# alan-turing-institute/rPSMF

Measured on AMD Instinct MI355X. Metric: PSMF filter timesteps/sec at d=100k r=32, higher is better.
Workload: dtype f64; 1 GPU; PSMF full filter, random-walk dynamics, d=100000 r=32 T=10000 synthetic Gaussian series, rows sharded over 1 GPU(s); d=100000, d_per_gpu=100000, r=32, T=10000, store_y_pred=True, engine=block

## Files before the change

rpsmf_amd/csrc/psmf_blk3.hip:

```cpp
#pragma once
#include "psmf_block.h"
#include "psmf_sweep.h"
#include "psmf_ns.hip"
#include "psmf_dyn.hip"
#include "psmf_wave.h"

namespace psmf {

constexpr int F3_NT = 512;
constexpr int F3_S = 34;
constexpr int F3_MAXIT = 12;

template <int MODE>
struct F3Mask {
  static constexpr bool full = MODE == 0;
  static constexpr bool small = MODE == 2;
  bool c1, r1[4], dg[4];
};
#define F3_VALID(mk, ti, tj, q) ((mk).full || ((mk).small ? ((ti) == 0 && (tj) == 0 && (mk).r1[q] && (mk).c1) \
                                                          : (((ti) == 0 || (mk).r1[q]) && ((tj) == 0 || (mk).c1))))
#define F3_DIAG(mk, ti, tj, q) (((ti) == (tj)) && (mk).dg[q])

enum { F3_KAPPA = 0, F3_N, F3_INVN, F3_EE, F3_IOM, F3_Q, F3_IQ, F3_PSCALE, F3_NSC = 16 };

// ... 12 lines not shown
  double* sc;
  double* nrm;
  double* hv;
  double* gp;
  double* tr;
  double* sab;
  double* sal;
  double* sbe;
  float* s32;
  double* rowbufX;
  double* rowbufY;
  int* errflag;
  long long* tick;
  long long* acc;
  long long* hand;
};

constexpr int F3_AS = 48;

inline size_t blk_filter3_lds_bytes() {
  const size_t doubles = (size_t)RB * RB + 2 * (size_t)RB * F3_AS + 2 * 32 * F3_S + 8 * RM + 2;
  return (doubles * 8 + 15) & ~(size_t)15;
}

struct F3Blk {
  long long k0;
  int nb, last;
  double* Acoef;
  double* Bcoef;
  const double* XG;
  const double* Aprev;
  int from_lds, to_lds;
};

enum { F3C_IQW = 0, F3C_IOM, F3C_PSCALE, F3C_Q, F3C_RHO, F3C_LAM, F3C_PHI, F3C_OMEGA, F3C_EE, F3C_S, F3C_ETA, F3C_N };
struct F3Carry {
  double* Xc;
  float* Xa;
  double* G;
  double* W;
  double* V;
  double* sc;
};
__device__ __forceinline__ F3Carry f3_carry(const F3Lds& L) {
  F3Carry c;
  c.Xc = L.dump;
  c.Xa = L.dumpP;
  c.G = L.dump + 4 * 8 * 64;
  c.W = L.dump + 6 * 8 * 64;
  c.V = L.img;
  c.sc = L.img + 16 * 64;
  return c;
}
__device__ __forceinline__ int f3_carry_xa(const int role, const int e, const int lane) { return (((e >> 3) * 4 + role) * 8 + (e & 7)) * 64 + lane; }

__device__ __forceinline__ void f3_ns_dump(DevState* st, const int role, const int lane, const double (&Xc)[8], const float (&Xa)[16],
                                           const double (&G)[16], const double (&Wf)[16], const double iq_w) {
#pragma unroll
  for (int e = 0; e < 8; ++e) st->f3_Xc[role][e * 64 + lane] = Xc[e];
#pragma unroll
  for (int e = 0; e < 16; ++e) st->f3_Xa[role][e * 64 + lane] = Xa[e];
  if (role == 0) {
#pragma unroll
    for (int e = 0; e < 16; ++e) st->f3_G[e * 64 + lane] = G[e];
    if (lane == 0) st->f3_sc[0] = iq_w;
  }
  if (role == 2) {
#pragma unroll
    for (int e = 0; e < 16; ++e) st->f3_W[e * 64 + lane] = Wf[e];
  }
}

__device__ __forceinline__ void f3_v0_dump(DevState* st, const F3Lds& L, const int r, const int lane, const long long kdone, const bool last,
                                           const double* V, const double* sc) {
  const int j = lane & 31, hf = lane >> 5;
  const double q = sc[F3C_Q];
#pragma unroll
  for (int t = 0; t < 16; ++t) st->f3_V[t * 64 + lane] = V[t];
  if (last) {
#pragma unroll
    for (int t = 0; t < 16; ++t) {
      const int i = 16 * hf + t;
      if (i < r && j < r) {
        st->V[i * r + j] = V[t];
        st->Q[i * r + j] = (i == j) ? q : 0.0;
      }
    }
  } else if (hf == 0 && j < r) {
    st->Q[j * r + j] = q;
  }
  if (lane < r) st->mu[lane] = L.mub[lane];
  if (lane == 0) {
    st->f3_sc[1] = sc[F3C_IOM]; st->f3_sc[2] = sc[F3C_PSCALE];
    st->k = kdone;
    st->rho = sc[F3C_RHO]; st->lam = sc[F3C_LAM]; st->phi = sc[F3C_PHI]; st->omega = sc[F3C_OMEGA]; st->ee = sc[F3C_EE];
    st->s_done = sc[F3C_S]; st->eta_done = sc[F3C_ETA]; st->N_done = sc[F3C_N];
    st->ns_valid = 3;
  }
}

__device__ __forceinline__ void f3_carry_flush(const BlockParams& b, const F3Lds& L, const long long kdone, const int tid) {
  DevState* st = b.sp.st;
  const int role = tid >> 6, lane = tid & 63;
  const F3Carry cy = f3_carry(L);
  if (role < 4) {
    double Xc[8], G[16], Wf[16];
    float Xa[16];
#pragma unroll
    for (int e = 0; e < 8; ++e) Xc[e] = cy.Xc[role * 512 + e * 64 + lane];
#pragma unroll
    for (int e = 0; e < 16; ++e) { Xa[e] = cy.Xa[f3_carry_xa(role, e, lane)]; G[e] = cy.G[e * 64 + lane]; Wf[e] = cy.W[e * 64 + lane]; }
    f3_ns_dump(st, role, lane, Xc, Xa, G, Wf, cy.sc[F3C_IQW]);
  } else if (role == 4) {
    double V[16], sc[12];
#pragma unroll
    for (int t = 0; t < 16; ++t) V[t] = cy.V[t * 64 + lane];
#pragma unroll
    for (int i = 0; i < 12; ++i) sc[i] = cy.sc[i];
    f3_v0_dump(st, L, b.sp.r, lane, kdone, false, V, sc);
  }
}

enum { F3A_CNT = 0, F3A_DUR = 4, F3A_GAP, F3A_TEND, F3A_BLOCKS, F3A_DBG = 8, F3A_BLK = 13, F3A_N = 17 };
__device__ __forceinline__ void f3_acc_flush(DevState* st, const long long* a) {
#pragma unroll
  for (int i = 0; i < 4; ++i) st->cnt[i] += a[F3A_CNT + i];
  st->cnt[4] += a[F3A_DUR];
  st->cnt[5] += a[F3A_GAP];
  st->cnt[6] = a[F3A_TEND];
  st->cnt[7] += a[F3A_BLOCKS];
#pragma unroll
  for (int i = 0; i < 5; ++i) st->dbg[i] += a[F3A_DBG + i];
  st->dbg[5] += 1;
}

__device__ __forceinline__ bool f3_chain_next(const BlockParams& b, const F3Lds& L, const long long seq) {
  asm volatile("s_waitcnt vmcnt(0)" ::: "memory");
  f3_barrier();
  if (__builtin_amdgcn_readfirstlane((int)L.hand[1]) != 0) {
    if (threadIdx.x == 6 * 64) flag_store(b.flags + 1, seq);
    return true;
  }
  return blk_chain_next(b, seq);
}

constexpr int F3_XS_TRIPS = RB * F3_AS / F3_NT;
constexpr int F3_AP_TRIPS = RB * 32 / F3_NT;
constexpr int F3_YY_TRIPS = 6;
static_assert(F3_XS_TRIPS * F3_NT == RB * F3_AS && F3_AP_TRIPS * F3_NT == RB * 32, "whole trips");
static_assert(F3_YY_TRIPS * (F3_NT / 64) >= F3_AS && F3_AS <= 64 && F3_AS <= XGB, "Y^T Y of the longest block");
struct F3XG {
  double xs[F3_XS_TRIPS], yy[F3_YY_TRIPS];
};
__device__ __forceinline__ void f3_xg_fetch(F3XG& x, const double* XG, const int nb, const int tid) {
#pragma unroll
  for (int u = 0; u < F3_YY_TRIPS; ++u) {
    const int q = max(min((tid >> 6) + 8 * u, nb - 1), 0), q2 = max(min(tid & 63, nb - 1), 0);
    x.yy[u] = xg_load(XG + (size_t)(RB + q) * XGB + q2);
  }
#pragma unroll
  for (int u = 0; u < F3_XS_TRIPS; ++u) {
    const int idx = tid + u * F3_NT, m = idx / F3_AS, q = idx - m * F3_AS;
    x.xs[u] = xg_load(XG + (size_t)m * XGB + max(min(q, nb - 1), 0));
  }
}
__device__ __forceinline__ void f3_xg_stage(const F3XG& x, double* sX, const int nb, const int tid) {
#pragma unroll
  for (int u = 0; u < F3_XS_TRIPS; ++u) {
    const int idx = tid + u * F3_NT, m = idx / F3_AS, q = idx - m * F3_AS;
    sX[m * F3_AS + q] = q < nb ? x.xs[u] : 0.0;
  }
}
__device__ __forceinline__ void f3_xg_corner(const F3XG& x, double* sK, const int r, const int nb, const int tid) {
#pragma unroll
  for (int u = 0; u < F3_YY_TRIPS; ++u) {
    const int q = (tid >> 6) + 8 * u, q2 = tid & 63;
    if (q < nb && q2 < nb) sK[(r + q) * RB + r + q2] = x.yy[u];
  }
}

__device__ __forceinline__ bool f3_xg_ahead(const F3Blk& k, const F3Lds& L, F3XG& x, const int tid) {
  if (__builtin_amdgcn_readfirstlane((int)L.hand[1]) == 0) return false;
  f3_xg_fetch(x, k.XG, k.nb, tid);
  f3_xg_stage(x, L.sKA, k.nb, tid);
  return true;
}

__device__ __forceinline__ void f3_assemble_K(const BlockParams& b, const F3Blk& k, const F3Lds& L, const int r, const int tid, F3XG& x,
                                              const bool ahead) {
  const int nb = k.nb, lane = tid & 63, w = tid >> 6, lrow = lane >> 4, lcol = lane & 15;
  double* sK = L.sK;
  double* sA = L.sA;
  double* sX = L.sA + RB * F3_AS;
  const DevState* st = b.sp.st;
  double gv[2];
#pragma unroll
  for (int u = 0; u < 2; ++u)
    gv[u] = k.from_lds ? f3_carry(L).G[(w + 8 * u) * 64 + lane]
                       : st->f3_G[(w + 8 * u) * 64 + lane];
  if (!ahead) f3_xg_fetch(x, k.XG, nb, tid);
  double ap[F3_AP_TRIPS];
  if (k.Aprev) {
#pragma unroll
    for (int u = 0; u < F3_AP_TRIPS; ++u) {
      const int idx = tid + u * F3_NT, m = idx >> 5, c = idx & 31;
      ap[u] = k.Aprev[m * r + min(c, r - 1)];
    }
  }
  if (r + nb < RB)
    for (int idx = tid; idx < RB * RB; idx += F3_NT) sK[idx] = 0.0;
  if (k.Aprev) {
#pragma unroll
    for (int u = 0; u < F3_AP_TRIPS; ++u) {
      const int idx = tid + u * F3_NT, m = idx >> 5, c = idx & 31;
      sA[m * F3_AS + c] = c < r ? ap[u] : 0.0;
    }
  }
  if (!ahead) {
    f3_xg_stage(x, sX, nb, tid);
    __syncthreads();
  } else if (r + nb < RB) {
    f3_barrier();
  }
#pragma unroll
  for (int u = 0; u < 2; ++u) {
    const int e = w + 8 * u;
    const int row = 16 * (e >> 3) + lrow + 4 * (e & 3), col = 16 * ((e >> 2) & 1) + lcol;
    if (row < r && col < r) sK[row * RB + col] = gv[u];
  }
  f3_xg_corner(x, sK, r, nb, tid);
  const int nct = (nb + 15) >> 4;
  if (w < 2 * nct) {
    const int ti = w & 1, ct = w >> 1;
    f64x4 acc = {0.0, 0.0, 0.0, 0.0};
#pragma unroll
    for (int kk = 0; kk < RB / 4; ++kk)
      acc = __builtin_amdgcn_mfma_f64_16x16x4f64(sA[(4 * kk + lrow) * F3_AS + 16 * ti + lcol], sX[(4 * kk + lrow) * F3_AS + 16 * ct + lcol], acc, 0, 0, 0);
#pragma unroll
    for (int q = 0; q < 4; ++q) {
      const int i = 16 * ti + lrow + 4 * q, c = 16 * ct + lcol;
      if (i < r && c < nb) { sK[i * RB + r + c] = acc[q]; sK[(r + c) * RB + i] = acc[q]; }
    }
  }
  f3_barrier();
}

#ifndef F3_KNOCK
#define F3_KNOCK 0
#endif
#ifndef F3_PREDICT
#define F3_PREDICT 1
#endif

template <int C, int FULL>
__device__ __forceinline__ double f3_ns_iter(const double (&Mf)[16], const double (&Xc)[8], const float (&Xa)[16], double (&Xn)[8],
                                             const F3Mask<FULL>& mk) {
  f64x4 acc[2] = {f64x4{0.0, 0.0, 0.0, 0.0}, f64x4{0.0, 0.0, 0.0, 0.0}};
#pragma unroll
  for (int kt = 0; kt < 2; ++kt)
#pragma unroll
    for (int kk = 0; kk < 4; ++kk)
#pragma unroll
      for (int ti = 0; ti < 2; ++ti)
        acc[ti] = __builtin_amdgcn_mfma_f64_16x16x4f64(Mf[(kt * 2 + ti) * 4 + kk], Xc[kt * 4 + kk], acc[ti], 0, 0, 0);
  double R[8];
  double nrm = 0.0;
#pragma unroll
  for (int ti = 0; ti < 2; ++ti)
#pragma unroll
    for (int q = 0; q < 4; ++q) {
      const double v = (F3_DIAG(mk, ti, C, q) ? 1.0 : 0.0) - acc[ti][q];
      R[ti * 4 + q] = v;
      nrm += v * v;
    }
  f32x4s d2[2] = {f32x4s{0.f, 0.f, 0.f, 0.f}, f32x4s{0.f, 0.f, 0.f, 0.f}};
  float Rf[8];
#pragma unroll
  for (int e = 0; e < 8; ++e) Rf[e] = (float)R[e];
#pragma unroll
  for (int kt = 0; kt < 2; ++kt)
#pragma unroll
    for (int kk = 0; kk < 4; ++kk)
#pragma unroll
      for (int to = 0; to < 2; ++to)
        if (!(F3_KNOCK & 512)) d2[to] = __builtin_amdgcn_mfma_f32_16x16x4f32(Xa[to * 8 + kt * 4 + kk], Rf[kt * 4 + kk], d2[to], 0, 0, 0);
#pragma unroll
  for (int to = 0; to < 2; ++to)
#pragma unroll
    for (int q = 0; q < 4; ++q) Xn[to * 4 + q] = Xc[to * 4 + q] + (double)d2[to][q];
  return nrm;
}

struct F3Ctl {
  bool have_prev;
  int ns_skip;
  int c_ns, c_sw, c_it, c_fail;
};
// ... 11 lines not shown
  nd.tq = nrm[10];
  return nd;
}
#define F3_DECIDE_FROM(nd_)                                                                                \
  do {                                                                                                     \
    const double nx_ = (nd_).nx[0] + (nd_).nx[1];                                                          \
    const double ny_ = (nd_).ny[0] + (nd_).ny[1];                                                          \
    const double worst_ = fmax(nx_, ny_);                                                                  \
    ++ctl.c_it;                                                                                            \
     \
     \
    if (worst_ < (nd_).tf[0]) done = true;         \
    else if (!(worst_ < (nd_).tf[1]) || it == F3_MAXIT - 1) failed = true;    \
       \
    else last = worst_ * worst_ < (nd_).tq;                                                                \
    if (F3_KNOCK & 1) { done = false; failed = false; last = true; }       \
  } while (0)
#define F3_DECIDE()                                                                                        \
  do {                                                                                                     \
    const F3Nrm nd_d_ = f3_norms_read(L.nrm, par);                                                         \
    F3_DECIDE_FROM(nd_d_);                                                                                 \
  } while (0)

__device__ __forceinline__ void f3_sweep_images(const F3Lds& L, const int r2, const int tid) {
  const int lt = tid & (WG - 1), c32 = lt & 31, rg = lt >> 5;
  const bool halfX = tid < WG;
  double* im = halfX ? L.img : L.img + 32 * F3_S;
  double A1[4];
#pragma unroll
  for (int m = 0; m < 4; ++m) A1[m] = im[(rg + 8 * m) * F3_S + c32];
  sweep_all<32>(A1, r2, c32, rg, halfX ? L.rowbufX : L.rowbufY, L.errflag);
#pragma unroll
  for (int m = 0; m < 4; ++m) {
    const int i = rg + 8 * m;
    if (i < r2 && c32 < r2) im[i * F3_S + c32] = -A1[m];
  }
  __syncthreads();
}

template <int C, int FULL>
__device__ __forceinline__ void f3_ns_program(const BlockParams& b, const F3Blk& k, const F3Lds& L, const int inv, const int role, const int lane,
                                              const bool carried) {
  const StepParams& p = b.sp;
  DevState* st = p.st;
  const int r = p.r, r2 = r + (r & 1), tid = 64 * role + lane;
  const int lrow = lane >> 4, lcol = lane & 15;
  const bool isX = inv == 0, isY = inv == 1;
  double* imgX = L.img;
  double* imgY = L.img + 32 * F3_S;
  double G[16], Wf[16], Xc[8];
  float Xa[16];
  const int pcol = (lcol >> 2) + 4 * (lcol & 3);
  const bool from_lds = k.from_lds != 0;
  const F3Carry cy = f3_carry(L);
  const double q0 = from_lds ? 0.0 : st->Q[0];
  F3Mask<FULL> mk;
  const int rt = FULL == 2 ? r : r - 16;
  mk.c1 = lcol < rt;
#pragma unroll
  for (int qq = 0; qq < 4; ++qq) { mk.r1[qq] = lrow + 4 * qq < rt; mk.dg[qq] = lcol == lrow + 4 * qq; }
#pragma unroll
  for (int ti = 0; ti < 2; ++ti)
#pragma unroll
    for (int tj = 0; tj < 2; ++tj)
#pragma unroll
      for (int qq = 0; qq < 4; ++qq) {
        const int row = 16 * ti + lrow + 4 * qq, col = 16 * tj + lcol;
        const bool in = row < r && col < r;
        const int e = (ti * 2 + tj) * 4 + qq;
        G[e] = in ? L.sK[row * RB + col] : 0.0;
        if (from_lds) {
          Wf[e] = cy.W[e * 64 + lane];
        } else if (carried) {
          Wf[e] = st->f3_W[e * 64 + lane];
        } else {
          const double l0 = imgX[row * F3_S + col];
          Wf[e] = in ? ((row == col ? q0 : 0.0) - q0 * q0 * l0) : 0.0;
        }
      }
#pragma unroll
  for (int e = 0; e < 8; ++e) {
    const int row = 16 * (e >> 2) + lrow + 4 * (e & 3);
    if (from_lds) Xc[e] = cy.Xc[role * 512 + e * 64 + lane];
    else Xc[e] = carried ? st->f3_Xc[role][e * 64 + lane] : (row == 16 * C + lcol ? 1.0 : 0.0);
  }
#pragma unroll
  for (int e = 0; e < 16; ++e) {
    const int row = 16 * ((e >> 2) & 1) + lrow + 4 * (e & 3), cp = 16 * (e >> 3) + pcol;
    if (from_lds) Xa[e] = cy.Xa[f3_carry_xa(role, e, lane)];
    else Xa[e] = carried ? st->f3_Xa[role][e * 64 + lane] : (row == cp ? 1.f : 0.f);
  }
  if (isX) {
    double g1 = 0.0, t1 = 0.0;
#pragma unroll
    for (int ti = 0; ti < 2; ++ti)
#pragma unroll
      for (int qq = 0; qq < 4; ++qq) {
        const int row = 16 * ti + lrow + 4 * qq, col = 16 * C + lcol;
        const bool in = row < r && col < r;
        const double g = G[(ti * 2 + C) * 4 + qq];
        double pv;
        if (carried) pv = Xc[ti * 4 + qq];
        else pv = st->P[in ? row * r + col : 0];
        g1 += in ? g * pv : 0.0;
        t1 += (row == col) ? g : 0.0;
      }
    g1 = wave_sum_f64_dpp(g1);
    t1 = wave_sum_f64_dpp(t1);
    if (lane == 0) { L.gp[C] = g1; L.tr[C] = t1; }
  }
  f3_barrier();

#define F3_W_AND_TRACES()                                                                                  \
  do {                                                                                                     \
    if (!(F3_KNOCK & 4))                                                                                   \
    _Pragma("unroll") for (int ti_ = 0; ti_ < 2; ++ti_)                                                    \
      _Pragma("unroll") for (int tj_ = 0; tj_ < 2; ++tj_) {                                                \
        double wv_[4];                                                                                     \
        if (isY && tj_ == C) {                                                                             \
          _Pragma("unroll") for (int q_ = 0; q_ < 4; ++q_) wv_[q_] = Xc[ti_ * 4 + q_];                     \
        } else if (w_from_img) {                                                                           \
          _Pragma("unroll") for (int q_ = 0; q_ < 4; ++q_) wv_[q_] = imgY[(16 * ti_ + lrow + 4 * q_) * F3_S + 16 * tj_ + lcol]; \
        } else {                                                                                           \
          const f64x2* d2_ = reinterpret_cast<const f64x2*>(L.dump) + (size_t)((w_par * 4 + 2 + tj_) * 4) * 64 + lane; \
          const f64x2 v0_ = d2_[(ti_ * 2) * 64], v1_ = d2_[(ti_ * 2 + 1) * 64];                            \
          wv_[0] = v0_[0]; wv_[1] = v0_[1]; wv_[2] = v1_[0]; wv_[3] = v1_[1];                               \
        }                                                                                                  \
        _Pragma("unroll") for (int q_ = 0; q_ < 4; ++q_)                                                   \
          Wf[(ti_ * 2 + tj_) * 4 + q_] = F3_VALID(mk, ti_, tj_, q_) ? wv_[q_] : 0.0;                       \
      }                                                                                                    \
    BLK_T(6);                                                                                              \
    if (isX && !(F3_KNOCK & 2)) {                                                                          \
      double g1_ = 0.0;                                                                                    \
      _Pragma("unroll") for (int ti_ = 0; ti_ < 2; ++ti_)                                                  \
        _Pragma("unroll") for (int q_ = 0; q_ < 4; ++q_)                                                   \
          g1_ += G[(ti_ * 2 + C) * 4 + q_] * Xc[ti_ * 4 + q_];                \
      g1_ = wave_sum_f64_dpp(g1_);                                                                         \
      if (lane == 0) L.gp[C] = g1_;                                                                        \
    } else if (isY && !(F3_KNOCK & 2)) {                                                                   \
       \
      double t1_ = 0.0;                                                                                    \
      _Pragma("unroll") for (int q_ = 0; q_ < 4; ++q_) t1_ += F3_DIAG(mk, C, C, q_) ? G[(C * 2 + C) * 4 + q_] : 0.0; \
      t1_ = wave_sum_f64_dpp(t1_);                                                                         \
// ... 188 lines not shown
      for (int ti = 0; ti < 2; ++ti)
#pragma unroll
        for (int qq = 0; qq < 4; ++qq) {
          const int row = 16 * ti + lrow + 4 * qq;
          Xc[ti * 4 + qq] = im[row * F3_S + 16 * C + lcol];
#pragma unroll
          for (int to = 0; to < 2; ++to) Xa[to * 8 + ti * 4 + qq] = (float)im[row * F3_S + 16 * to + pcol];
        }
    } else {
      ++ctl.c_ns;
    }
    ctl.have_prev = true;
    w_par = par;
    w_from_img = from_img;
    if (!(F3_KNOCK & 8)) {
      double vp0 = 0.0, vp1 = 0.0, vq0 = 0.0, vq1 = 0.0;
#pragma unroll
      for (int qq = 0; qq < 4; ++qq) {
        vp0 += Xc[qq] * hrow[qq]; vp1 += Xc[4 + qq] * hrow[4 + qq];
        vq0 += Xc[qq] * wrow[qq]; vq1 += Xc[4 + qq] * wrow[4 + qq];
      }
      const double vp = xor32_sum_f64(xor16_sum_f64(vp0 + vp1));
      int lane_f = lane;
      asm volatile("" : "+v"(lane_f));
      const int lcol = lane_f & 15, lrow = lane_f >> 4;
      const int j = 16 * C + lcol;
      if (isX) {
        const double mu_new = mub_j + kap_k * vp;
        if (lrow == 0 && j < r) {
          L.mub[j] = mu_new;
          if (p.mu_hist) p.mu_hist[(size_t)(k.k0 + jb + 1 - p.series_t0) * r + j] = mu_new;
        }
        if (p.robust) {
          const double hvp = wave_sum_f64_dpp((lrow == 0) ? h_j * vp : 0.0);
          if (lane == 0) L.hv[C] = hvp;
        }
      }
      if (F3_PREDICT && (p.ns_predict & 1)) {
        const double vq = xor32_sum_f64(xor16_sum_f64(vq0 + vq1));
        if (lrow == 0) *reinterpret_cast<f64x2*>(L.sab + 2 * (32 * inv + j)) = f64x2{vp, vq};
      }
      smw_ok = true;
    }
    BLK_T(5);
    f3_barrier();
    BLK_T(1);
  }
  BLK_TOUT();
  if (fetch_late) F3_FETCH_PARTNER(w_par);
  if (k.nb > 0) F3_W_AND_TRACES();
  f3_barrier();
  const double ps = L.sc[F3_PSCALE], iom = L.sc[F3_IOM];
  if (k.to_lds) {
#pragma unroll
    for (int e = 0; e < 8; ++e) cy.Xc[role * 512 + e * 64 + lane] = Xc[e];
#pragma unroll
    for (int e = 0; e < 16; ++e) cy.Xa[f3_carry_xa(role, e, lane)] = Xa[e];
    if (role == 0) {
#pragma unroll
      for (int e = 0; e < 16; ++e) cy.G[e * 64 + lane] = G[e];
      if (lane == 0) cy.sc[F3C_IQW] = iq_w;
    }
    if (role == 2) {
#pragma unroll
      for (int e = 0; e < 16; ++e) cy.W[e * 64 + lane] = Wf[e];
    }
  } else {
    f3_ns_dump(st, role, lane, Xc, Xa, G, Wf, iq_w);
  }
  if (k.last) {
#pragma unroll
    for (int ti = 0; ti < 2; ++ti)
#pragma unroll
      for (int qq = 0; qq < 4; ++qq) {
        const int row = 16 * ti + lrow + 4 * qq, col = 16 * C + lcol;
        if (row < r && col < r) {
          const int idx = row * r + col;
          if (isX) {
            st->XpX[idx] = Xc[ti * 4 + qq];
            st->P[idx] = ps * Xc[ti * 4 + qq];
            st->G[idx] = G[(ti * 2 + C) * 4 + qq];
          } else {
            st->XpY[idx] = Xc[ti * 4 + qq];
            st->Lbar[idx] = ((row == col ? iq_w : 0.0) - Wf[(ti * 2 + C) * 4 + qq] * iq_w * iq_w) * iom;
          }
        }
      }
  }
  if (role == 0 && lane == 0) { L.acc[F3A_BLK] = ctl.c_ns; L.acc[F3A_BLK + 1] = ctl.c_sw; L.acc[F3A_BLK + 2] = ctl.c_it; L.acc[F3A_BLK + 3] = ctl.c_fail; }
#undef F3_ITERATE
#undef F3_FETCH_PARTNER
#undef F3_W_AND_TRACES
}

template <int ROLE>
__device__ __forceinline__ void f3_v_program(const BlockParams& b, const F3Blk& k, const F3Lds& L, const int lane, const bool carried) {
  const StepParams& p = b.sp;
  DevState* st = p.st;
  constexpr int role = ROLE;
  const int r = p.r, r2 = r + (r & 1), tid = 64 * role + lane;
  const double dd = (double)p.d, idd = 1.0 / dd;
  constexpr bool isV0 = ROLE == 4, isV1 = ROLE == 5, isV2 = ROLE == 6, isV3 = ROLE == 7;
  __builtin_amdgcn_s_setprio(3);
  double pr[32];
#pragma unroll
  for (int i = 0; i < 32; ++i) pr[i] = 0.0;
  double kappa = 0.0, Nk = 0.0, invN = 0.0, s_k = 0.0, eta_k = 0.0, ee_k = 0.0, phi = 1.0, omega = 1.0, pscale = 1.0, wj = 0.0;
  const bool from_lds = k.from_lds != 0;
  const F3Carry cy = f3_carry(L);
  double q, rho, lam;
  if (from_lds) { q = cy.sc[F3C_Q]; rho = cy.sc[F3C_RHO]; lam = cy.sc[F3C_LAM]; }
  else { q = st->Q[0]; rho = st->rho; lam = st->lam; }
  double iom0 = 1.0;
  double kap7 = 1.0;
  if (isV0) {
    const int j = lane & 31, hf = lane >> 5;
    if (from_lds) {
#pragma unroll
      for (int t = 0; t < 16; ++t) pr[t] = cy.V[t * 64 + lane];
      iom0 = cy.sc[F3C_IOM];
      pscale = cy.sc[F3C_PSCALE];
    } else if (carried) {
#pragma unroll
      for (int t = 0; t < 16; ++t) pr[t] = st->f3_V[t * 64 + lane];
      iom0 = st->f3_sc[1];
      pscale = st->f3_sc[2];
    } else {
#pragma unroll
      for (int t = 0; t < 16; ++t) {
        const int i = 16 * hf + t;
        const bool in = i < r && j < r;
        const double v = st->V[in ? i * r + j : 0];
        pr[t] = in ? v : 0.0;
      }
    }
  } else if (isV1) {
#pragma unroll
    for (int c = 0; c < 32; ++c) pr[c] = (lane == c && c < r) ? 1.0 : 0.0;
  } else if (isV2) {
#pragma unroll
    for (int c = 0; c < 32; ++c) pr[c] = (c < r) ? L.sK[lane * RB + c] : 0.0;
  } else {
    const int c = lane & 31, hf = lane >> 5;
#pragma unroll
    for (int t = 0; t < 32; ++t) pr[t] = (32 * hf + t == c && c < r) ? 1.0 : 0.0;
  }
  f3_barrier();

#define F3_V0_FINISH_PREV()                                               \
  do {                                                                    \
    omega = 1.0;                                                          \
    pscale = 1.0;                                                         \
    if (p.robust) {                                                       \
      const double hPh_ = L.hv[0] + L.hv[1];                              \
      const double quad_ = kappa * ee_k - kappa * kappa * hPh_;           \
      omega = (lam + quad_) * fast_rcp(lam + dd);                         \
      pscale = p.beta * omega;                                            \
      rho *= omega;                                                       \
      q *= omega;                                                         \
      if (!p.fixed_lambda) lam += dd;                                     \
    }                                                                     \
  } while (0)

  F3Ctl ctl = {carried, 0, 0, 0, 0, 0};
  if (role == 4 && lane == 0) L.tick[0] = (long long)__builtin_amdgcn_s_memrealtime();
  BLK_T0();
  for (int jb = 0; jb < k.nb; ++jb) {
    const bool poll = isV2 && k.to_lds && jb == k.nb - 1;
    long long poll_xg = 0, poll_ab = 1;
    if (poll) { poll_xg = flag_load(b.flags + 0); poll_ab = flag_load(b.flags + 2); }
    double cm = 0.0;
    if (isV0 && !(F3_KNOCK & 1024)) {
// ... 77 lines not shown
    } else if (isV1) {
      const double e1 = wave_sum_f64_dpp(cm * L.Ka[lane]);
      if (lane == 0) L.sc[F3_EE] = e1;
    } else if (isV0) {
      wj = xor32_sum_f64(wj);
      if (lane < 32) L.w[lane] = wj;
      const double gpv = pscale * (L.gp[0] + L.gp[1]) + q * (L.tr[0] + L.tr[1]);
      eta_k = rho + gpv * idd;
      Nk = s_k + eta_k;
      invN = fast_rcp(Nk);
      if (lane == 0) { L.sc[F3_N] = Nk; L.sc[F3_INVN] = invN; }
    }
    BLK_T(2);
    f3_barrier();
    BLK_T(1);
    bool done = false, failed = !try_ns, last = false;
    int it = 0;
    const F3Nrm nd0 = f3_norms_read(L.nrm, 0);
    if (F3_KNOCK & 128) {
    } else if (isV3) {
      const int c = lane & 31, hf = lane >> 5;
      const double wn = L.w[c] * L.sc[F3_INVN];
#pragma unroll
      for (int t = 0; t < 32; ++t) pr[t] += L.a[32 * hf + t] * wn;
    } else if (isV1 || isV2) {
      const double cn = cm * L.sc[F3_INVN];
#pragma unroll
      for (int c = 0; c < 32; ++c) pr[c] += cn * L.w[c];
    } else if (isV0) {
      const int hf = lane >> 5;
      ee_k = L.sc[F3_EE];
      phi = 1.0;
      double vscale = 1.0;
      if (p.robust) {
        phi = (lam + ee_k * invN) * fast_rcp(lam + dd);
        vscale = p.alpha * phi;
      }
      const double wjn = wj * invN;
#pragma unroll
      for (int t = 0; t < 16; ++t) pr[t] = vscale * (pr[t] - L.w[16 * hf + t] * wjn);
    }
#pragma unroll
    for (int t = 0; t < (isV0 ? 16 : 32); t += 8)
      asm volatile("" : "+v"(pr[t]), "+v"(pr[t + 1]), "+v"(pr[t + 2]), "+v"(pr[t + 3]), "+v"(pr[t + 4]), "+v"(pr[t + 5]), "+v"(pr[t + 6]), "+v"(pr[t + 7]));
    if (try_ns) {
      F3_DECIDE_FROM(nd0);
      if (!done && !failed) {
        par = 1;
        it = 1;
        if (last) done = true;
      }
    }
    if (poll && lane == 0) L.hand[1] = (poll_ab == 0 && poll_xg >= L.hand[0]) ? 1 : 0;
    BLK_T(3);
    if (!done) {
      f3_barrier();
      while (try_ns && !done && !failed) {
        F3_DECIDE();
        if (done || failed) break;
        par ^= 1;
        ++it;
        if (last) { done = true; break; }
        f3_barrier();
      }
    }
    if (!done) {
      if (try_ns) { ++ctl.c_fail; ctl.ns_skip = p.ns_skip_n; }
      ++ctl.c_sw;
      f3_barrier();
      f3_sweep_images(L, r2, tid);
    } else {
      ++ctl.c_ns;
    }
    ctl.have_prev = true;
    BLK_T(4);
    f3_barrier();
    BLK_T(1);
  }
  BLK_TOUT();
  if (role == 4 && lane == 0) L.tick[1] = (long long)__builtin_amdgcn_s_memrealtime();

  if (isV0) {
    if (k.nb > 0) F3_V0_FINISH_PREV();
    if (lane == 0) { L.sc[F3_PSCALE] = pscale; L.sc[F3_IOM] = fast_rcp(omega); L.sc[F3_Q] = q; }
  } else if (isV1) {
#pragma unroll
    for (int c = 0; c < 32; ++c) L.sA[lane * F3_AS + c] = pr[c];
  }
  f3_barrier();
  if (isV0) {
    double sc[12];
    sc[F3C_IQW] = 0.0; sc[F3C_IOM] = L.sc[F3_IOM]; sc[F3C_PSCALE] = pscale; sc[F3C_Q] = q; sc[F3C_RHO] = rho; sc[F3C_LAM] = lam;
    sc[F3C_PHI] = phi; sc[F3C_OMEGA] = omega; sc[F3C_EE] = ee_k; sc[F3C_S] = s_k; sc[F3C_ETA] = eta_k; sc[F3C_N] = Nk;
    if (k.to_lds) {
#pragma unroll
      for (int t = 0; t < 16; ++t) cy.V[t * 64 + lane] = pr[t];
      if (lane == 0) {
#pragma unroll
        for (int i = 1; i < 12; ++i) cy.sc[i] = sc[i];
      }
    } else {
      f3_v0_dump(st, L, r, lane, k.k0 + k.nb, k.last != 0, pr, sc);
    }
    if (lane == 0 && *L.errflag && st->err == 0) st->err = (int)(k.k0 + 1);
  }
  for (int idx = tid - 256; idx < RB * r; idx += 256) { const int m = idx / r, c = idx - m * r; coef_store(k.Acoef + idx, L.sA[m * F3_AS + c]); }
#undef F3_V0_FINISH_PREV
}

}
```

rpsmf_amd/csrc/psmf_blk34.hip:

```cpp
#pragma once
#include "psmf_blk3.hip"
#include "psmf_blk4.hip"

namespace psmf {

template <bool SMALL, int KIND = 0>
__device__ __forceinline__ void blk_filter3_body(const BlockParams& b0) {
  extern __shared__ __attribute__((aligned(16))) char smem_raw[];
  double* sm = reinterpret_cast<double*>(smem_raw);
  const StepParams& p = b0.sp;
  DevState* st = p.st;
  const int r = p.r, tid0 = threadIdx.x;
  const int r2 = r + (r & 1);
  __shared__ __attribute__((aligned(16))) double hot[2 * 4 * 8 * 64 + 3 * RM + 2 * RB + F3_NSC + 12 + 6 + 8 * 32];
  __shared__ __attribute__((aligned(16))) float hotP[2 * 4 * 2 * 64 * 4];
  __shared__ __attribute__((aligned(16))) float hotS[2 * 128];
  F3Lds L;
  L.sK = sm;
  L.sA = L.sK + RB * RB;
  L.sKA = L.sA + RB * F3_AS;
  L.img = L.sKA + RB * F3_AS;
  L.rowbufX = L.img + 2 * 32 * F3_S;
  L.rowbufY = L.rowbufX + 4 * RM;
  L.errflag = reinterpret_cast<int*>(L.rowbufY + 4 * RM);
  L.dump = hot;
  L.dumpP = hotP;
  L.mub = L.dump + 2 * 4 * 8 * 64;
  L.w = L.mub + RM;
  L.h = L.w + RM;
  L.a = L.h + RM;
  L.Ka = L.a + RB;
  L.sc = L.Ka + RB;
  L.nrm = L.sc + F3_NSC;
  L.hv = L.nrm + 12;
  L.gp = L.hv + 2;
  L.tr = L.gp + 2;
  L.sab = L.tr + 2;
  L.sal = L.sab + 128;
  L.sbe = L.sal + 64;
  L.s32 = hotS;
  __shared__ long long s_tick[2];
  L.tick = s_tick;
  __shared__ long long s_acc[F3A_N];
  __shared__ long long s_hand[2];
  L.acc = s_acc;
  L.hand = s_hand;
  __shared__ __attribute__((aligned(16))) double hot4[KIND >= 1 ? 5 * RM + 2 * 48 + F4_NKC : 2];
  F4Lds D;
  D.fd = hot4; D.mu = D.fd + RM; D.tp = D.mu + RM; D.th = D.tp + RM; D.rs = D.th + 2 * RM; D.qs = D.rs + 48; D.kc = D.qs + 48;
  if (tid0 == 0) { L.nrm[8] = p.ns_tol2; L.nrm[9] = p.ns_far2; L.nrm[10] = 0.25 * p.ns_tol2; }

  const int nchain = b0.chain > 1 ? b0.chain : 1;
  const bool carry = KIND == 0 && b0.chain > 1 && b0.carry != 0;
  const bool acc_lds = b0.chain > 1;
  if (tid0 == 0) {
#pragma unroll
    for (int i = 0; i < F3A_N; ++i) s_acc[i] = 0;
    if (acc_lds) s_acc[F3A_TEND] = st->cnt[6];
    s_hand[1] = 0;
  }
  for (int j = 0; j < nchain; ++j) {
  int tid = tid0;
  asm volatile("" : "+v"(tid));
  const int lane = tid & 63;
  const int role = __builtin_amdgcn_readfirstlane(tid >> 6);
  const BlockParams& b = b0;
  F3Blk k;
  k.k0 = b0.k0; k.nb = b0.nb; k.last = b0.last; k.Acoef = b0.Acoef; k.Bcoef = b0.Bcoef; k.XG = b0.XG; k.Aprev = b0.Aprev;
  k.from_lds = (carry && j > 0) ? 1 : 0;
  k.to_lds = (carry && j < nchain - 1) ? 1 : 0;
  int assemble = b0.assemble;
  long long seq = b0.seq;
  if (b0.chain > 1) {
    const int slot = j & 1;
    k.k0 = b0.k0 + (long long)j * b0.chain_B;
    const long long left = b0.chain_kend - k.k0;
    k.nb = (int)(left < b0.chain_B ? left : b0.chain_B);
    k.Acoef = b0.Acoef0 + (size_t)slot * RB * RM;
    k.Bcoef = b0.Bcoef0 + (size_t)slot * RB * RB;
    seq = b0.seq + j;
    k.last = (j == nchain - 1) ? b0.last : 0;
    if (j > 0) {
      assemble = 1;
      k.XG = b0.XG0 + (size_t)slot * (RB + XGB) * XGB;
      k.Aprev = nullptr;
    }
  }
  const long long t_begin = (long long)__builtin_amdgcn_s_memrealtime();
  F3XG xg = {};
  bool ahead = false;
  if (j > 0) {
    if (carry && b0.xg_ahead) ahead = f3_xg_ahead(k, L, xg, tid);
    if (!(carry ? f3_chain_next(b0, L, seq) : blk_chain_next(b0, seq))) {
      if (k.from_lds) f3_carry_flush(b0, L, k.k0, tid);
      if (tid == 0) f3_acc_flush(st, L.acc);
      return;
    }
  } else {
    double pf = 0.0;
    if (b.flags) {
      if (assemble) {
        pf = k.XG[(size_t)tid * 16];
        if (tid < RB * RM / 16) pf += k.Aprev[tid * 16];
      }
      constexpr int kDumpLines = (int)((sizeof(st->f3_G) + sizeof(st->f3_W) + sizeof(st->f3_Xc) + sizeof(st->f3_V) + sizeof(st->f3_Xa)) / 128);
      static_assert(kDumpLines <= F3_NT, "one line per thread");
      if (tid < kDumpLines) pf += st->f3_G[tid * 16];
    }
    if (!blk_handoff_begin(b)) return;
    if (pf == 1.2345e300) hot[0] = pf;
  }
  const long long t_h = (long long)__builtin_amdgcn_s_memrealtime();
  if (!assemble) {
    for (int idx = tid; idx < RB * RB; idx += F3_NT) L.sK[idx] = b.K[idx];
  } else {
    f3_assemble_K(b, k, L, r, tid, xg, ahead);
  }
  if (tid == 0) { *L.errflag = 0; L.hand[0] = seq + 1; L.hand[1] = 0; L.acc[F3A_BLK] = 0; L.acc[F3A_BLK + 1] = 0; L.acc[F3A_BLK + 2] = 0; L.acc[F3A_BLK + 3] = 0; }
  const bool warm = KIND == 1 && j > 0;
  if (tid < RM) {
    if (!k.from_lds) L.mub[tid] = (tid < r && KIND == 0) ? st->mu[tid] : 0.0;
    if (!warm) { L.w[tid] = 0.0; L.h[tid] = 0.0; }
  }
  if (tid < F3_NSC && !warm) L.sc[tid] = 0.0;
  if (KIND >= 1) {
    if (tid < RM) { D.mu[tid] = (tid < r) ? st->mu[tid] : 0.0; D.fd[tid] = 0.0; D.tp[tid] = 0.0; }
    if (tid >= 64 && tid < 64 + 2 * RM) {
      const int i = tid - 64, j = i & (RM - 1), hi = i >> 6;
      const bool phased = p.dyn_kind == DYN_SINUSOID && (p.dyn_flags & 2);
      const bool have = p.n_theta > 0 && j < r && (hi == 0 || phased);
      const double tv = p.theta[have ? hi * r + j : 0];
      D.th[i] = have ? tv : 0.0;
    }
    if (tid >= 320 && tid < 320 + F4_NKC) f4_fill_trig_constants(D.kc, tid - 320);
    if (tid >= 256 && tid < 256 + 48) {
      const int jb_ = tid - 256;
      const long long ks = min((long long)(k.k0 + jb_ + 1), (long long)(k.k0 + k.nb)) - p.series_t0;
      if (p.rho_sched) D.rs[jb_] = p.rho_sched[ks];
      if (p.q_sched) D.qs[jb_] = p.q_sched[ks];
    }
  }
  const bool carried = k.from_lds ? true : st->ns_valid == (KIND == 2 ? 5 : (KIND == 1 ? 4 : 3));
  f3_barrier();
  const long long t_a = (long long)__builtin_amdgcn_s_memrealtime();
  if (!carried && KIND == 0) {
    const int lt = tid & (WG - 1), c32 = lt & 31, rg = lt >> 5;
    double* im = tid < WG ? L.img : L.img + 32 * F3_S;
    const double q0 = st->Q[0];
#pragma unroll
    for (int m = 0; m < 4; ++m) {
      const int i = rg + 8 * m;
      const bool in = (i < r) && (c32 < r);
      const double pv = st->P[in ? i * r + c32 : 0];
      im[i * F3_S + c32] = in ? pv + (i == c32 ? q0 : 0.0) : (i == c32 ? 1.0 : 0.0);
    }
    __syncthreads();
    f3_sweep_images(L, r2, tid);
  }
  if (KIND == 2) {
    if (role < 4) f5_idle_program(k);
    else if (role == 4) f5_v_program<4>(b, k, L, D, lane, carried);
    else if (role == 5) f5_v_program<5>(b, k, L, D, lane, carried);
    else if (role == 6) f5_v_program<6>(b, k, L, D, lane, carried);
    else f5_v_program<7>(b, k, L, D, lane, carried);
  } else if (KIND == 1) {
    const int md = SMALL ? 2 : (r == 32 ? 0 : 1);
    if (role < 2) {
      if (md == 2) { if (role & 1) f4_x_program<1, 2>(b, k, L, D, role, lane, carried, warm && carried); else f4_x_program<0, 2>(b, k, L, D, role, lane, carried, warm && carried); }
      else if (md == 0) { if (role & 1) f4_x_program<1, 0>(b, k, L, D, role, lane, carried, warm && carried); else f4_x_program<0, 0>(b, k, L, D, role, lane, carried, warm && carried); }
      else { if (role & 1) f4_x_program<1, 1>(b, k, L, D, role, lane, carried, warm && carried); else f4_x_program<0, 1>(b, k, L, D, role, lane, carried, warm && carried); }
    } else if (role < 4) {
      if (md == 2) { if (role & 1) f4_y_program<1, 2>(b, k, L, D, role, lane, carried, warm && carried); else f4_y_program<0, 2>(b, k, L, D, role, lane, carried, warm && carried); }
      else if (md == 0) { if (role & 1) f4_y_program<1, 0>(b, k, L, D, role, lane, carried, warm && carried); else f4_y_program<0, 0>(b, k, L, D, role, lane, carried, warm && carried); }
      else { if (role & 1) f4_y_program<1, 1>(b, k, L, D, role, lane, carried, warm && carried); else f4_y_program<0, 1>(b, k, L, D, role, lane, carried, warm && carried); }
    } else {
      if (role == 4) f4_v_program<4>(b, k, L, D, lane, carried, warm && carried);
      else if (role == 5) f4_v_program<5>(b, k, L, D, lane, carried, warm && carried);
      else if (role == 6) f4_v_program<6>(b, k, L, D, lane, carried, warm && carried);
      else f4_v_program<7>(b, k, L, D, lane, carried, warm && carried);
    }
  } else if (role < 4) {
    const int inv = role >> 1;
    if (SMALL) {
      if (role & 1) f3_ns_program<1, 2>(b, k, L, inv, role, lane, carried);
      else f3_ns_program<0, 2>(b, k, L, inv, role, lane, carried);
    } else if (r == 32) {
      if (role & 1) f3_ns_program<1, 0>(b, k, L, inv, role, lane, carried);
      else f3_ns_program<0, 0>(b, k, L, inv, role, lane, carried);
    } else if (r > 16) {
      if (role & 1) f3_ns_program<1, 1>(b, k, L, inv, role, lane, carried);
      else f3_ns_program<0, 1>(b, k, L, inv, role, lane, carried);
    }
  } else {
    if (role == 4) f3_v_program<4>(b, k, L, lane, carried);
    else if (role == 5) f3_v_program<5>(b, k, L, lane, carried);
    else if (role == 6) f3_v_program<6>(b, k, L, lane, carried);
    else f3_v_program<7>(b, k, L, lane, carried);
  }
  if (tid == 0) {
    const long long t_end = (long long)__builtin_amdgcn_s_memrealtime();
    const long long dt[5] = {t_h - t_begin, t_a - t_h, L.tick[0] - t_a, L.tick[1] - L.tick[0], t_end - L.tick[1]};
    if (acc_lds) {
      long long* a = L.acc;
#pragma unroll
      for (int i = 0; i < 4; ++i) a[F3A_CNT + i] += a[F3A_BLK + i];
#pragma unroll
      for (int i = 0; i < 5; ++i) a[F3A_DBG + i] += dt[i];
      a[F3A_DUR] += t_end - t_begin;
      if (a[F3A_TEND] != 0) a[F3A_GAP] += t_begin - a[F3A_TEND];
      a[F3A_TEND] = t_end;
      a[F3A_BLOCKS] += 1;
    } else {
#pragma unroll
      for (int i = 0; i < 4; ++i) st->cnt[i] += L.acc[F3A_BLK + i];
#pragma unroll
      for (int i = 0; i < 5; ++i) st->dbg[i] += dt[i];
      st->cnt[4] += t_end - t_begin;
      if (st->cnt[6] != 0) st->cnt[5] += t_begin - st->cnt[6];
      st->cnt[6] = t_end;
      st->cnt[7] += 1;
      if (j == 0) st->dbg[5] += 1;
    }
  }
  }
  if (b0.chain > 1) {
    asm volatile("s_waitcnt vmcnt(0)" ::: "memory");
    __syncthreads();
    if (tid0 == 0) {
      flag_store(b0.flags + 1, b0.seq + nchain);
      f3_acc_flush(st, s_acc);
    }
  }
}

__global__ __launch_bounds__(F3_NT) void psmf_blk_filter3(BlockParams b0) { blk_filter3_body<false>(b0); }
__global__ __launch_bounds__(F3_NT) void psmf_blk_filter3s(BlockParams b0) { blk_filter3_body<true>(b0); }
__global__ __launch_bounds__(F3_NT) void psmf_blk_filter4(BlockParams b0) { blk_filter3_body<false, 1>(b0); }
__global__ __launch_bounds__(F3_NT) void psmf_blk_filter4s(BlockParams b0) { blk_filter3_body<true, 1>(b0); }
__global__ __launch_bounds__(F3_NT) void psmf_blk_filter5(BlockParams b0) { blk_filter3_body<false, 2>(b0); }

}
```

Before: 333,300 timesteps/s.

## Use wide interleaved LDS carry layout and drop a barrier in block chaining

For the full-rank (non-small) KIND 0 path, the LDS carry buffers (Xc, Xa, G, W, V) switch to an interleaved layout so each lane moves them with 128-bit vector loads and stores instead of scalar ones. When the carry comes from LDS, the barrier at the end of K assembly is skipped and the hand[1] reset is elided. The Acoef store is moved earlier, uses incremental index arithmetic instead of per-element division, and the sA fill happens inside the last block iteration. Per-block accumulator bookkeeping is spread across a wave's lanes instead of running serially on thread 0. The trade-off is reliance on subtle ordering assumptions once the barrier is removed, which risks races.

```diff
diff --git a/rpsmf_amd/csrc/psmf_blk3.hip b/rpsmf_amd/csrc/psmf_blk3.hip
--- a/rpsmf_amd/csrc/psmf_blk3.hip
+++ b/rpsmf_amd/csrc/psmf_blk3.hip
@@ -88,7 +88,12 @@
   c.sc = L.img + 16 * 64;
   return c;
 }
-__device__ __forceinline__ int f3_carry_xa(const int role, const int e, const int lane) { return (((e >> 3) * 4 + role) * 8 + (e & 7)) * 64 + lane; }
+template <bool WIDE>
+__device__ __forceinline__ int f3_carry_d(const int e, const int lane) { return WIDE ? (e >> 1) * 128 + 2 * lane + (e & 1) : e * 64 + lane; }
+template <bool WIDE>
+__device__ __forceinline__ int f3_carry_xa(const int role, const int e, const int lane) {
+  return WIDE ? ((((e >> 3) * 4 + role) * 2 + ((e >> 2) & 1)) * 64 + lane) * 4 + (e & 3) : (((e >> 3) * 4 + role) * 8 + (e & 7)) * 64 + lane;
+}
 
 __device__ __forceinline__ void f3_ns_dump(DevState* st, const int role, const int lane, const double (&Xc)[8], const float (&Xa)[16],
                                            const double (&G)[16], const double (&Wf)[16], const double iq_w) {
@@ -135,6 +140,7 @@
   }
 }
 
+template <bool WIDE>
 __device__ __forceinline__ void f3_carry_flush(const BlockParams& b, const F3Lds& L, const long long kdone, const int tid) {
   DevState* st = b.sp.st;
   const int role = tid >> 6, lane = tid & 63;
@@ -143,14 +149,14 @@
     double Xc[8], G[16], Wf[16];
     float Xa[16];
 #pragma unroll
-    for (int e = 0; e < 8; ++e) Xc[e] = cy.Xc[role * 512 + e * 64 + lane];
-#pragma unroll
-    for (int e = 0; e < 16; ++e) { Xa[e] = cy.Xa[f3_carry_xa(role, e, lane)]; G[e] = cy.G[e * 64 + lane]; Wf[e] = cy.W[e * 64 + lane]; }
+    for (int e = 0; e < 8; ++e) Xc[e] = cy.Xc[role * 512 + f3_carry_d<WIDE>(e, lane)];
+#pragma unroll
+    for (int e = 0; e < 16; ++e) { Xa[e] = cy.Xa[f3_carry_xa<WIDE>(role, e, lane)]; G[e] = cy.G[f3_carry_d<WIDE>(e, lane)]; Wf[e] = cy.W[f3_carry_d<WIDE>(e, lane)]; }
     f3_ns_dump(st, role, lane, Xc, Xa, G, Wf, cy.sc[F3C_IQW]);
   } else if (role == 4) {
     double V[16], sc[12];
 #pragma unroll
-    for (int t = 0; t < 16; ++t) V[t] = cy.V[t * 64 + lane];
+    for (int t = 0; t < 16; ++t) V[t] = cy.V[f3_carry_d<WIDE>(t, lane)];
 #pragma unroll
     for (int i = 0; i < 12; ++i) sc[i] = cy.sc[i];
     f3_v0_dump(st, L, b.sp.r, lane, kdone, false, V, sc);
@@ -222,8 +228,9 @@
   return true;
 }
 
+template <bool WIDE>
 __device__ __forceinline__ void f3_assemble_K(const BlockParams& b, const F3Blk& k, const F3Lds& L, const int r, const int tid, F3XG& x,
-                                              const bool ahead) {
+                                              const bool ahead, const bool close) {
   const int nb = k.nb, lane = tid & 63, w = tid >> 6, lrow = lane >> 4, lcol = lane & 15;
   double* sK = L.sK;
   double* sA = L.sA;
@@ -232,7 +239,7 @@
   double gv[2];
 #pragma unroll
   for (int u = 0; u < 2; ++u)
-    gv[u] = k.from_lds ? f3_carry(L).G[(w + 8 * u) * 64 + lane]
+    gv[u] = k.from_lds ? f3_carry(L).G[f3_carry_d<WIDE>(w + 8 * u, lane)]
                        : st->f3_G[(w + 8 * u) * 64 + lane];
   if (!ahead) f3_xg_fetch(x, k.XG, nb, tid);
   double ap[F3_AP_TRIPS];
@@ -278,7 +285,19 @@
       if (i < r && c < nb) { sK[i * RB + r + c] = acc[q]; sK[(r + c) * RB + i] = acc[q]; }
     }
   }
-  f3_barrier();
+  if (!WIDE || close) f3_barrier();
+}
+
+__device__ __forceinline__ void f3_store_Acoef(double* Acoef, const double* sA, const int r, const int t) {
+  const float ir = __builtin_amdgcn_rcpf((float)r);
+  const int qs = __builtin_amdgcn_readfirstlane(256 / r), cs = 256 - qs * r, as = qs * F3_AS + cs;
+  const int m = (int)(((float)t + 0.5f) * ir);
+  int c = t - m * r, at = m * F3_AS + c;
+  for (int idx = t; idx < RB * r; idx += 256) {
+    coef_store(Acoef + idx, sA[at]);
+    c += cs; at += as;
+    if (c >= r) { c -= r; at += F3_AS - r; }
+  }
 }
 
 #ifndef F3_KNOCK
@@ -396,6 +415,7 @@
   float Xa[16];
   const int pcol = (lcol >> 2) + 4 * (lcol & 3);
   const bool from_lds = k.from_lds != 0;
+  constexpr bool WIDE = FULL != 2;
   const F3Carry cy = f3_carry(L);
   const double q0 = from_lds ? 0.0 : st->Q[0];
   F3Mask<FULL> mk;
@@ -414,7 +434,7 @@
         const int e = (ti * 2 + tj) * 4 + qq;
         G[e] = in ? L.sK[row * RB + col] : 0.0;
         if (from_lds) {
-          Wf[e] = cy.W[e * 64 + lane];
+          if (!WIDE) Wf[e] = cy.W[e * 64 + lane];
         } else if (carried) {
           Wf[e] = st->f3_W[e * 64 + lane];
         } else {
@@ -425,14 +445,28 @@
 #pragma unroll
   for (int e = 0; e < 8; ++e) {
     const int row = 16 * (e >> 2) + lrow + 4 * (e & 3);
-    if (from_lds) Xc[e] = cy.Xc[role * 512 + e * 64 + lane];
+    if (from_lds) { if (!WIDE) Xc[e] = cy.Xc[role * 512 + e * 64 + lane]; }
     else Xc[e] = carried ? st->f3_Xc[role][e * 64 + lane] : (row == 16 * C + lcol ? 1.0 : 0.0);
   }
 #pragma unroll
   for (int e = 0; e < 16; ++e) {
     const int row = 16 * ((e >> 2) & 1) + lrow + 4 * (e & 3), cp = 16 * (e >> 3) + pcol;
-    if (from_lds) Xa[e] = cy.Xa[f3_carry_xa(role, e, lane)];
+    if (from_lds) { if (!WIDE) Xa[e] = cy.Xa[f3_carry_xa<false>(role, e, lane)]; }
     else Xa[e] = carried ? st->f3_Xa[role][e * 64 + lane] : (row == cp ? 1.f : 0.f);
+  }
+  if (WIDE && from_lds) {
+    const f64x2* w2 = reinterpret_cast<const f64x2*>(cy.W) + lane;
+    const f64x2* x2 = reinterpret_cast<const f64x2*>(cy.Xc + role * 512) + lane;
+    const f32x4s* a4 = reinterpret_cast<const f32x4s*>(cy.Xa) + lane;
+#pragma unroll
+    for (int e = 0; e < 16; e += 2) { const f64x2 v = w2[(e >> 1) * 64]; Wf[e] = v[0]; Wf[e + 1] = v[1]; }
+#pragma unroll
+    for (int e = 0; e < 8; e += 2) { const f64x2 v = x2[(e >> 1) * 64]; Xc[e] = v[0]; Xc[e + 1] = v[1]; }
+#pragma unroll
+    for (int e = 0; e < 16; e += 4) {
+      const f32x4s v = a4[f3_carry_xa<true>(role, e, 0) >> 2];
+      Xa[e] = v[0]; Xa[e + 1] = v[1]; Xa[e + 2] = v[2]; Xa[e + 3] = v[3];
+    }
   }
   if (isX) {
     double g1 = 0.0, t1 = 0.0;
@@ -727,18 +761,38 @@
   f3_barrier();
   const double ps = L.sc[F3_PSCALE], iom = L.sc[F3_IOM];
   if (k.to_lds) {
-#pragma unroll
-    for (int e = 0; e < 8; ++e) cy.Xc[role * 512 + e * 64 + lane] = Xc[e];
-#pragma unroll
-    for (int e = 0; e < 16; ++e) cy.Xa[f3_carry_xa(role, e, lane)] = Xa[e];
-    if (role == 0) {
-#pragma unroll
-      for (int e = 0; e < 16; ++e) cy.G[e * 64 + lane] = G[e];
-      if (lane == 0) cy.sc[F3C_IQW] = iq_w;
-    }
-    if (role == 2) {
-#pragma unroll
-      for (int e = 0; e < 16; ++e) cy.W[e * 64 + lane] = Wf[e];
+    if (WIDE) {
+      f64x2* x2 = reinterpret_cast<f64x2*>(cy.Xc + role * 512) + lane;
+      f32x4s* a4 = reinterpret_cast<f32x4s*>(cy.Xa) + lane;
+#pragma unroll
+      for (int e = 0; e < 8; e += 2) x2[(e >> 1) * 64] = f64x2{Xc[e], Xc[e + 1]};
+#pragma unroll
+      for (int e = 0; e < 16; e += 4) a4[f3_carry_xa<true>(role, e, 0) >> 2] = f32x4s{Xa[e], Xa[e + 1], Xa[e + 2], Xa[e + 3]};
+      if (role == 0) {
+        f64x2* g2 = reinterpret_cast<f64x2*>(cy.G) + lane;
+#pragma unroll
+        for (int e = 0; e < 16; e += 2) g2[(e >> 1) * 64] = f64x2{G[e], G[e + 1]};
+        if (lane == 0) cy.sc[F3C_IQW] = iq_w;
+      }
+      if (role == 2) {
+        f64x2* w2 = reinterpret_cast<f64x2*>(cy.W) + lane;
+#pragma unroll
+        for (int e = 0; e < 16; e += 2) w2[(e >> 1) * 64] = f64x2{Wf[e], Wf[e + 1]};
+      }
+    } else {
+#pragma unroll
+      for (int e = 0; e < 8; ++e) cy.Xc[role * 512 + e * 64 + lane] = Xc[e];
+#pragma unroll
+      for (int e = 0; e < 16; ++e) cy.Xa[f3_carry_xa<false>(role, e, lane)] = Xa[e];
+      if (role == 0) {
+#pragma unroll
+        for (int e = 0; e < 16; ++e) cy.G[e * 64 + lane] = G[e];
+        if (lane == 0) cy.sc[F3C_IQW] = iq_w;
+      }
+      if (role == 2) {
+#pragma unroll
+        for (int e = 0; e < 16; ++e) cy.W[e * 64 + lane] = Wf[e];
+      }
     }
   } else {
     f3_ns_dump(st, role, lane, Xc, Xa, G, Wf, iq_w);
@@ -768,7 +822,7 @@
 #undef F3_W_AND_TRACES
 }
 
-template <int ROLE>
+template <int ROLE, bool WIDE>
 __device__ __forceinline__ void f3_v_program(const BlockParams& b, const F3Blk& k, const F3Lds& L, const int lane, const bool carried) {
   const StepParams& p = b.sp;
   DevState* st = p.st;
@@ -792,7 +846,10 @@
     const int j = lane & 31, hf = lane >> 5;
     if (from_lds) {
 #pragma unroll
-      for (int t = 0; t < 16; ++t) pr[t] = cy.V[t * 64 + lane];
+      for (int t = 0; t < 16; t += 2) {
+        if (WIDE) { const f64x2 v = reinterpret_cast<const f64x2*>(cy.V)[(t >> 1) * 64 + lane]; pr[t] = v[0]; pr[t + 1] = v[1]; }
+        else { pr[t] = cy.V[t * 64 + lane]; pr[t + 1] = cy.V[(t + 1) * 64 + lane]; }
+      }
       iom0 = cy.sc[F3C_IOM];
       pscale = cy.sc[F3C_PSCALE];
     } else if (carried) {
@@ -976,6 +1033,10 @@
       }
     }
     if (poll && lane == 0) L.hand[1] = (poll_ab == 0 && poll_xg >= L.hand[0]) ? 1 : 0;
+    if (WIDE && isV1 && jb == k.nb - 1) {
+#pragma unroll
+      for (int c = 0; c < 32; ++c) L.sA[lane * F3_AS + c] = pr[c];
+    }
     BLK_T(3);
     if (!done) {
       f3_barrier();
@@ -1004,10 +1065,11 @@
   BLK_TOUT();
   if (role == 4 && lane == 0) L.tick[1] = (long long)__builtin_amdgcn_s_memrealtime();
 
+  if (WIDE) f3_store_Acoef(k.Acoef, L.sA, r, tid - 256);
   if (isV0) {
     if (k.nb > 0) F3_V0_FINISH_PREV();
     if (lane == 0) { L.sc[F3_PSCALE] = pscale; L.sc[F3_IOM] = fast_rcp(omega); L.sc[F3_Q] = q; }
-  } else if (isV1) {
+  } else if (!WIDE && isV1) {
 #pragma unroll
     for (int c = 0; c < 32; ++c) L.sA[lane * F3_AS + c] = pr[c];
   }
@@ -1018,7 +1080,10 @@
     sc[F3C_PHI] = phi; sc[F3C_OMEGA] = omega; sc[F3C_EE] = ee_k; sc[F3C_S] = s_k; sc[F3C_ETA] = eta_k; sc[F3C_N] = Nk;
     if (k.to_lds) {
 #pragma unroll
-      for (int t = 0; t < 16; ++t) cy.V[t * 64 + lane] = pr[t];
+      for (int t = 0; t < 16; t += 2) {
+        if (WIDE) reinterpret_cast<f64x2*>(cy.V)[(t >> 1) * 64 + lane] = f64x2{pr[t], pr[t + 1]};
+        else { cy.V[t * 64 + lane] = pr[t]; cy.V[(t + 1) * 64 + lane] = pr[t + 1]; }
+      }
       if (lane == 0) {
 #pragma unroll
         for (int i = 1; i < 12; ++i) cy.sc[i] = sc[i];
@@ -1028,7 +1093,7 @@
     }
     if (lane == 0 && *L.errflag && st->err == 0) st->err = (int)(k.k0 + 1);
   }
-  for (int idx = tid - 256; idx < RB * r; idx += 256) { const int m = idx / r, c = idx - m * r; coef_store(k.Acoef + idx, L.sA[m * F3_AS + c]); }
+  if (!WIDE) for (int idx = tid - 256; idx < RB * r; idx += 256) { const int m = idx / r, c = idx - m * r; coef_store(k.Acoef + idx, L.sA[m * F3_AS + c]); }
 #undef F3_V0_FINISH_PREV
 }
 
diff --git a/rpsmf_amd/csrc/psmf_blk34.hip b/rpsmf_amd/csrc/psmf_blk34.hip
--- a/rpsmf_amd/csrc/psmf_blk34.hip
+++ b/rpsmf_amd/csrc/psmf_blk34.hip
@@ -52,6 +52,7 @@
 
   const int nchain = b0.chain > 1 ? b0.chain : 1;
   const bool carry = KIND == 0 && b0.chain > 1 && b0.carry != 0;
+  constexpr bool WIDE = KIND == 0 && !SMALL;
   const bool acc_lds = b0.chain > 1;
   if (tid0 == 0) {
 #pragma unroll
@@ -92,7 +93,7 @@
   if (j > 0) {
     if (carry && b0.xg_ahead) ahead = f3_xg_ahead(k, L, xg, tid);
     if (!(carry ? f3_chain_next(b0, L, seq) : blk_chain_next(b0, seq))) {
-      if (k.from_lds) f3_carry_flush(b0, L, k.k0, tid);
+      if (k.from_lds) f3_carry_flush<WIDE>(b0, L, k.k0, tid);
       if (tid == 0) f3_acc_flush(st, L.acc);
       return;
     }
@@ -111,12 +112,17 @@
     if (pf == 1.2345e300) hot[0] = pf;
   }
   const long long t_h = (long long)__builtin_amdgcn_s_memrealtime();
+  const bool one_barrier = WIDE && k.from_lds != 0;
   if (!assemble) {
     for (int idx = tid; idx < RB * RB; idx += F3_NT) L.sK[idx] = b.K[idx];
   } else {
-    f3_assemble_K(b, k, L, r, tid, xg, ahead);
-  }
-  if (tid == 0) { *L.errflag = 0; L.hand[0] = seq + 1; L.hand[1] = 0; L.acc[F3A_BLK] = 0; L.acc[F3A_BLK + 1] = 0; L.acc[F3A_BLK + 2] = 0; L.acc[F3A_BLK + 3] = 0; }
+    f3_assemble_K<WIDE>(b, k, L, r, tid, xg, ahead, !one_barrier);
+  }
+  if (tid == 0) {
+    *L.errflag = 0; L.hand[0] = seq + 1;
+    if (!one_barrier) L.hand[1] = 0;
+    L.acc[F3A_BLK] = 0; L.acc[F3A_BLK + 1] = 0; L.acc[F3A_BLK + 2] = 0; L.acc[F3A_BLK + 3] = 0;
+  }
   const bool warm = KIND == 1 && j > 0;
   if (tid < RM) {
     if (!k.from_lds) L.mub[tid] = (tid < r && KIND == 0) ? st->mu[tid] : 0.0;
@@ -192,12 +198,31 @@
       else f3_ns_program<0, 1>(b, k, L, inv, role, lane, carried);
     }
   } else {
-    if (role == 4) f3_v_program<4>(b, k, L, lane, carried);
-    else if (role == 5) f3_v_program<5>(b, k, L, lane, carried);
-    else if (role == 6) f3_v_program<6>(b, k, L, lane, carried);
-    else f3_v_program<7>(b, k, L, lane, carried);
-  }
-  if (tid == 0) {
+    if (role == 4) f3_v_program<4, WIDE>(b, k, L, lane, carried);
+    else if (role == 5) f3_v_program<5, WIDE>(b, k, L, lane, carried);
+    else if (role == 6) f3_v_program<6, WIDE>(b, k, L, lane, carried);
+    else f3_v_program<7, WIDE>(b, k, L, lane, carried);
+  }
+  if (WIDE && acc_lds) {
+    if (role == 0) {
+      static_assert(F3A_CNT == 0 && F3A_DUR == 4 && F3A_GAP == 5 && F3A_TEND == 6 && F3A_BLOCKS == 7 && F3A_DBG == 8 && F3A_BLK == 13, "one lane per word of F3Lds::acc");
+      const long long t_end = (long long)__builtin_amdgcn_s_memrealtime();
+      long long* a = L.acc;
+      const int wd = lane < F3A_BLK ? lane : 0;
+      const long long tk0 = L.tick[0], tk1 = L.tick[1], tend0 = a[F3A_TEND], old = a[wd], blk = a[F3A_BLK + (lane & 3)];
+      long long add = blk;
+      if (wd == F3A_DUR) add = t_end - t_begin;
+      if (wd == F3A_GAP) add = tend0 != 0 ? t_begin - tend0 : 0;
+      if (wd == F3A_TEND) add = t_end - old;
+      if (wd == F3A_BLOCKS) add = 1;
+      if (wd == F3A_DBG) add = t_h - t_begin;
+      if (wd == F3A_DBG + 1) add = t_a - t_h;
+      if (wd == F3A_DBG + 2) add = tk0 - t_a;
+      if (wd == F3A_DBG + 3) add = tk1 - tk0;
+      if (wd == F3A_DBG + 4) add = t_end - tk1;
+      if (lane < F3A_BLK) a[wd] = old + add;
+    }
+  } else if (tid == 0) {
     const long long t_end = (long long)__builtin_amdgcn_s_memrealtime();
     const long long dt[5] = {t_h - t_begin, t_a - t_h, L.tick[0] - t_a, L.tick[1] - L.tick[0], t_end - L.tick[1]};
     if (acc_lds) {
```

Measured after the change: 341,700 timesteps/s, median of 6. 2.5% higher.
